# linnanwang/FastGen

Measured on AMD Instinct MI355X. Metric: images/sec at 4-step distilled (DMD2) sampling, higher is better.
Workload: dtype fp32 (tensors, accumulate) with split-bf16 x3 MFMA conv products; 1 GPU; EDM CIFAR-10 32x32 SongUNet (55.7M params) DMD2 4-step 'sde' sampling, batch=512 per GPU; global_batch=512, sample_steps=4, parallelism=replicas x1 (no data-path collective), graph=True

## Files before the change

### fastgen_amd/csrc/conv.h

```cpp
#pragma once
#include <hip/hip_runtime.h>

struct ConvArgs {
    const void* src1;
    const void* src2;
    int C1, C2;
    int Hs, Ws;
    int H, W;
    int B;
    const float2* ab;
    const void* wpack;
    const void* wpack_ws;
    const float* bias;
    const float* temb;
    int temb_stride;
    const void* resid;
    float scale;
    void* out;
    int Cout;
    float2* stats;
    int dbg;
    void* q_out;
    void* k_out;
    void* vt_out;
    const float* gate = nullptr;
    int gate_stride = 0;
    int act = 0;
    int heads = 0, head_dim = 0;
    size_t heads_lo_off = 0;
};

enum { PRO_NONE = 0, PRO_GN = 1, PRO_GN_SILU = 2 };
enum { RES_NONE = 0, RES_DOWN = 1, RES_UP = 2 };
enum { OUT_NHWC = 0, OUT_QKV = 1, OUT_TOK = 2, OUT_HEADS = 3 };

int launch_conv_fused(int dtype, int ks, int pro, int res, int outmode, const ConvArgs& a, hipStream_t stream);
int conv_stat_slots(int W);
bool conv_ws_supported(int dtype, int ks, int pro, int res, int outmode, const ConvArgs& a);
bool conv_ws_enabled();
int launch_conv_ws(int res, const ConvArgs& a, hipStream_t stream, bool prepare_only, int pro = PRO_GN_SILU);
bool conv_ws_shape_ok(int dtype, int cout, int cin, int res);
int launch_pack_conv_weights_ws(const float* w_oihw, void* wpack_ws, int cout, int cin, hipStream_t stream);
bool conv_x3ws_supported(int ks, int pro, int res, int outmode, const ConvArgs& a);
bool conv_x3ws_shape_ok(int cout, int cin, int res);
int conv_x3ws_stat_slots(int W);
int launch_conv_x3ws(int res, const ConvArgs& a, hipStream_t stream, bool prepare_only, int pro = PRO_GN_SILU);
int launch_pack_conv_weights_x3ws(const float* w_oihw, void* wpack_ws, int cout, int cin, hipStream_t stream);
int conv_launch_stat_slots(int dtype, int ks, int pro, int res, int outmode, const ConvArgs& a);
int launch_conv_ws_debug(const ConvArgs& a, int abl, hipStream_t stream);
int launch_conv_debug(int dtype, const ConvArgs& a, hipStream_t stream);
int conv_prepare_all(int dtype);
size_t conv_pack_elems(int cout, int cin, int ks);
int launch_pack_conv_weights(int dtype, const float* w_oihw, void* wpack, int cout, int cin, int ks, int qkv_perm,
                             hipStream_t stream);
```

### fastgen_amd/csrc/conv_ws3.hip

```cpp
#include "common.h"
#include "conv.h"

namespace {

constexpr int X3_NTHR = 768;
constexpr int X3_KC = 32;
constexpr int X3_PA = 16;
constexpr int X3_PLANE = 3072;
constexpr int X3_ABUF = 8 * X3_PLANE;
constexpr int X3_RING = 4;
constexpr int X3_HOFF = 128 * 512;
constexpr int X3_LDS = X3_HOFF + X3_RING * X3_ABUF;
constexpr int X3_STEPB = 9 * 2048;

template <int LOGW>
struct X3Geom {
    static constexpr int W = 1 << LOGW;
    static constexpr int TW = 16, TH = 8;
    static constexpr int TCOLS = W / TW;
    static constexpr int TPI = (W / TH) * TCOLS;
    static constexpr int HW_ = TW + 2, HH_ = TH + 2;
    static constexpr int HALO_PIX = HW_ * HH_;
    static constexpr int RS = HW_ * X3_PA;
};

__device__ __forceinline__ void x3_barrier() {
    asm volatile("s_waitcnt lgkmcnt(0)\n\ts_barrier" ::: "memory");
}

struct X3Frag {
    bf16x8 hi, lo;
};

template <int RES, int LOGW, int PRO>
__global__ __launch_bounds__(X3_NTHR) void conv3_x3ws_kernel(const ConvArgs a, const int ntiles) {
    using G = X3Geom<LOGW>;
    extern __shared__ __attribute__((aligned(16))) char smem[];
    char* const hbuf = smem;
    char* const ring = smem + X3_HOFF;

    const int tid = threadIdx.x;
    const int lane = tid & 63;
    const int wave = __builtin_amdgcn_readfirstlane(tid >> 6);
    const int Cin = a.C1 + a.C2;
    const int nchunk = Cin / X3_KC;
    const int G8 = (int)gridDim.x >> 3;
    const int wg = ((gridDim.x & 7) == 0) ? ((int)blockIdx.x & 7) * G8 + ((int)blockIdx.x >> 3) : (int)blockIdx.x;
    const int gstride = (int)gridDim.x;
    const int my_tiles = (ntiles - wg + gstride - 1) / gstride;
    const int S = my_tiles * nchunk;
    const int NSTEP = S + 3;
    const int H = a.H;

    if (wave < 8) {
        const int grp = wave >> 2, wl = wave & 3;
        const int col = lane & 15, g4 = lane >> 4;
        const size_t wstride = (size_t)nchunk * 9 * 1024;
        const __amdgpu_buffer_rsrc_t wrs = __builtin_amdgcn_make_buffer_rsrc(
            const_cast<__bf16*>(reinterpret_cast<const __bf16*>(a.wpack_ws) + (size_t)(grp * 8 + wl * 2) * wstride), 0, 0x7fffffff,
            0x00020000);
        const int wvoff = lane * 16;
        const int wsb = (int)(wstride * 2);
        auto load_w = [&](int byte_off) -> X3Frag {
            X3Frag f;
            f.hi = __builtin_bit_cast(bf16x8, __builtin_amdgcn_raw_buffer_load_b128(wrs, wvoff, byte_off, 0));
            f.lo = __builtin_bit_cast(bf16x8, __builtin_amdgcn_raw_buffer_load_b128(wrs, wvoff, byte_off + 1024, 0));
            return f;
        };
        X3Frag wq[3][2];
#pragma unroll
        for (int j = 0; j < 3; ++j)
#pragma unroll
            for (int nt = 0; nt < 2; ++nt) wq[j][nt] = load_w(nt * wsb + j * 2048);

        f32x4 acc[8][2];
#pragma unroll
        for (int m = 0; m < 8; ++m)
#pragma unroll
            for (int nt = 0; nt < 2; ++nt) acc[m][nt] = f32x4{0.f, 0.f, 0.f, 0.f};

        const int lane_off = g4 * X3_PLANE + col * X3_PA;
        const int dl0 = col * 512 + ((8 * wl + ((g4) ^ (col & 7))) << 4);
        const int dl1 = col * 512 + ((8 * wl + ((4 + g4) ^ (col & 7))) << 4);

        x3_barrier();
        int c = 0;
        for (int s = 0; s < NSTEP; ++s) {
            const int ls = s - 2 * grp;
            if (ls >= 0 && ls < S) {
                const char* abase = ring + (ls & 3) * X3_ABUF + lane_off;
                const int cn = (c + 1 == nchunk) ? 0 : c + 1;
                const int wcur = c * X3_STEPB;
                const int wnxt = (ls + 1 < S) ? cn * X3_STEPB : wcur;
                auto read_x = [&](int q, X3Frag (&xf)[2]) {
                    const int tap = q >> 2, m0 = 2 * (q & 3);
                    const int off = (tap / 3 + m0) * G::RS + (tap % 3) * X3_PA;
#pragma unroll
                    for (int m = 0; m < 2; ++m) {
                        xf[m].hi = *reinterpret_cast<const bf16x8*>(abase + off + m * G::RS);
                        xf[m].lo = *reinterpret_cast<const bf16x8*>(abase + off + m * G::RS + 4 * X3_PLANE);
                    }
                };
                auto mma12 = [&](int q, const X3Frag (&xf)[2]) {
                    const int tap = q >> 2, m0 = 2 * (q & 3);
                    const X3Frag(&wf)[2] = wq[tap % 3];
#pragma unroll
                    for (int m = 0; m < 2; ++m)
#pragma unroll
                        for (int nt = 0; nt < 2; ++nt)
                            acc[m0 + m][nt] = __builtin_amdgcn_mfma_f32_16x16x32_bf16(wf[nt].hi, xf[m].lo, acc[m0 + m][nt], 0, 0, 0);
#pragma unroll
                    for (int m = 0; m < 2; ++m)
#pragma unroll
                        for (int nt = 0; nt < 2; ++nt)
                            acc[m0 + m][nt] = __builtin_amdgcn_mfma_f32_16x16x32_bf16(wf[nt].lo, xf[m].hi, acc[m0 + m][nt], 0, 0, 0);
#pragma unroll
                    for (int m = 0; m < 2; ++m)
#pragma unroll
                        for (int nt = 0; nt < 2; ++nt)
                            acc[m0 + m][nt] = __builtin_amdgcn_mfma_f32_16x16x32_bf16(wf[nt].hi, xf[m].hi, acc[m0 + m][nt], 0, 0, 0);
                    if ((q & 3) != 3) return;
                    const int pn = (tap + 3 < 9) ? wcur + (tap + 3) * 2048 : wnxt + (tap + 3 - 9) * 2048;
#pragma unroll
                    for (int nt = 0; nt < 2; ++nt) wq[tap % 3][nt] = load_w(pn + nt * wsb);
                };
                X3Frag x0[2], x1[2];
                read_x(0, x0);
#pragma unroll
                for (int q = 0; q < 36; q += 2) {
                    read_x(q + 1, x1);
                    __builtin_amdgcn_sched_barrier(0);
                    mma12(q, x0);
                    __builtin_amdgcn_sched_barrier(0);
                    if (q + 2 < 36) read_x(q + 2, x0);
                    __builtin_amdgcn_sched_barrier(0);
                    mma12(q + 1, x1);
                    __builtin_amdgcn_sched_barrier(0);
                }
                if (c + 1 == nchunk) {
#pragma unroll
                    for (int m = 0; m < 8; ++m) {
                        *reinterpret_cast<f32x4*>(hbuf + m * 8192 + dl0) = acc[m][0];
                        *reinterpret_cast<f32x4*>(hbuf + m * 8192 + dl1) = acc[m][1];
                        acc[m][0] = f32x4{0.f, 0.f, 0.f, 0.f};
                        acc[m][1] = f32x4{0.f, 0.f, 0.f, 0.f};
                    }
                }
                c = cn;
            }
            x3_barrier();
        }
        return;
    }

    const int ptid = tid - 512;
    const int pw = wave - 8;
    const int oct = ptid & 3;
    const float* src1 = reinterpret_cast<const float*>(a.src1);
    const float* src2 = reinterpret_cast<const float*>(a.src2);
    int hdy[3], hdx[3], hlds[3];
#pragma unroll
    for (int i = 0; i < 3; ++i) {
        const int hq = min((ptid >> 2) + 64 * i, G::HALO_PIX - 1);
        const int hy = hq / G::HW_, hx = hq - hy * G::HW_;
        hdy[i] = hy - 1;
        hdx[i] = hx - 1;
        hlds[i] = oct * X3_PLANE + hy * G::RS + hx * X3_PA;
    }
    const bool third = (ptid >> 2) + 128 < G::HALO_PIX;

    auto tile_coord = [&](int t, int& n, int& slot, int& row0, int& col0) {
        n = t / G::TPI;
        slot = t - n * G::TPI;
        row0 = (slot / G::TCOLS) * G::TH;
        col0 = (slot % G::TCOLS) * G::TW;
    };

    struct Staged {
        f32x4 raw[3][2];
        float2 ab[8];
    };
    unsigned off1[3], off2[3];
    bool valid[3];
    const float2* abn = a.ab;
    auto tile_setup = [&](int t) __attribute__((always_inline)) {
        int n, slot, row0, col0;
        tile_coord(t, n, slot, row0, col0);
#pragma unroll
        for (int i = 0; i < 3; ++i) {
            const int y = row0 + hdy[i], x = col0 + hdx[i];
            valid[i] = (y >= 0) && (y < H) && (x >= 0) && (x < G::W) && (i < 2 || third);
            const int yc = min(max(y, 0), H - 1), xc = min(max(x, 0), G::W - 1);
            const int sy = (RES == RES_UP) ? (yc >> 1) : yc, sx = (RES == RES_UP) ? (xc >> 1) : xc;
            const unsigned pix = (unsigned)((n * a.Hs + sy) * a.Ws + sx);
            off1[i] = (pix * (unsigned)a.C1 + oct * 8) * 4u;
            off2[i] = (pix * (unsigned)a.C2 + oct * 8) * 4u;
        }
        abn = a.ab + (size_t)n * Cin;
    };
    auto stage_load = [&](Staged& st, int t, int c32) __attribute__((always_inline)) {
        if (c32 == 0) tile_setup(t);
        const bool first = c32 * X3_KC < a.C1;
        const char* base = first ? reinterpret_cast<const char*>(src1) + c32 * (X3_KC * 4)
                                 : reinterpret_cast<const char*>(src2) + (c32 * X3_KC - a.C1) * 4;
#pragma unroll
        for (int i = 0; i < 3; ++i) {
            const char* p = base + (first ? off1[i] : off2[i]);
            st.raw[i][0] = *reinterpret_cast<const f32x4*>(p);
            st.raw[i][1] = *reinterpret_cast<const f32x4*>(p + 16);
        }
        if (PRO == PRO_NONE) return;
        const float2* p = abn + c32 * X3_KC + oct * 8;
#pragma unroll
        for (int j = 0; j < 8; j += 2) {
            const f32x4 q = *reinterpret_cast<const f32x4*>(p + j);
            st.ab[j] = make_float2(q[0], q[1]);
            st.ab[j + 1] = make_float2(q[2], q[3]);
        }
    };
    auto stage_store = [&](const Staged& st, char* abuf) __attribute__((always_inline)) {
#pragma unroll
        for (int i = 0; i < 3; ++i) {
            float v[8];
#pragma unroll
            for (int j = 0; j < 8; ++j) {
                v[j] = st.raw[i][j >> 2][j & 3];
                if (PRO != PRO_NONE) v[j] = silu_f<true>(fmaf(v[j], st.ab[j].x, st.ab[j].y));
            }
            bf16x8 hi, lo;
            split8(v, hi, lo);
            typedef __attribute__((ext_vector_type(4))) unsigned u32x4;
            u32x4 wh = __builtin_bit_cast(u32x4, hi), wl_ = __builtin_bit_cast(u32x4, lo);
#pragma unroll
            for (int j = 0; j < 4; ++j) {
                wh[j] = valid[i] ? wh[j] : 0u;
                wl_[j] = valid[i] ? wl_[j] : 0u;
            }
            if (i < 2 || third) {
                *reinterpret_cast<u32x4*>(abuf + hlds[i]) = wh;
                *reinterpret_cast<u32x4*>(abuf + hlds[i] + 4 * X3_PLANE) = wl_;
            }
        }
    };

    const int chq = lane & 31, psub = lane >> 5;
    float* const out = reinterpret_cast<float*>(a.out);
    const float* const resid = reinterpret_cast<const float*>(a.resid);
    const bool has_resid = __builtin_amdgcn_readfirstlane(resid != nullptr);
    auto retire_half = [&](int t, int half) __attribute__((always_inline)) {
        int n, slot, row0, col0;
        tile_coord(t, n, slot, row0, col0);
        const int co = half * 128 + chq * 4;
        f32x4 radd = {0.f, 0.f, 0.f, 0.f};
        if (a.bias) radd = *reinterpret_cast<const f32x4*>(a.bias + co);
        if (a.temb) radd += *reinterpret_cast<const f32x4*>(a.temb + (size_t)n * a.temb_stride + co);
        radd *= a.scale;
        const size_t tb = (((size_t)n * H + row0) * G::W + col0) * 256 + co;
        float ssum = 0.f, ssq = 0.f;
#pragma unroll 1
        for (int grp8 = 0; grp8 < 2; ++grp8) {
            f32x4 rr[8], dv[8];
            unsigned go[8];
#pragma unroll
            for (int j = 0; j < 8; ++j) {
                const int px = pw * 32 + 2 * (grp8 * 8 + j) + psub;
                go[j] = (unsigned)(((px >> 4) * G::W + (px & 15)) * 256);
                rr[j] = f32x4{0.f, 0.f, 0.f, 0.f};
                if (has_resid) rr[j] = *reinterpret_cast<const f32x4*>(resid + tb + go[j]);
                dv[j] = *reinterpret_cast<const f32x4*>(hbuf + px * 512 + ((chq ^ (px & 7)) << 4));
            }
#pragma unroll
            for (int j = 0; j < 8; ++j) {
                f32x4 v;
#pragma unroll
                for (int e = 0; e < 4; ++e) v[e] = fmaf(dv[j][e], a.scale, radd[e]);
                if (has_resid) {
#pragma unroll
                    for (int e = 0; e < 4; ++e) v[e] = fmaf(rr[j][e], a.scale, v[e]);
                }
                *reinterpret_cast<f32x4*>(out + tb + go[j]) = v;
                ssum += (v[0] + v[1]) + (v[2] + v[3]);
                ssq += (v[0] * v[0] + v[1] * v[1]) + (v[2] * v[2] + v[3] * v[3]);
            }
        }
        ssum += __shfl_xor(ssum, 32);
        ssq += __shfl_xor(ssq, 32);
        if (a.stats && psub == 0) a.stats[(((size_t)n * G::TPI + slot) * 4 + pw) * 64 + half * 32 + chq] = make_float2(ssum, ssq);
    };

    auto advance = [&](int& t, int& cc) {
        if (++cc == nchunk) {
            cc = 0;
            t += gstride;
        }
    };
    Staged st;
    int t1 = wg, c1 = 0;
    stage_load(st, t1, c1);
    stage_store(st, ring);
    advance(t1, c1);
    x3_barrier();
    int sa = 0;
    for (int s = 0; s < NSTEP; ++s) {
        const bool more = s + 1 < S;
        if (more) stage_load(st, t1, c1);
        if (sa == 0 && s >= nchunk && s <= S) retire_half(wg + (s / nchunk - 1) * gstride, 0);
        if (sa == 2 % nchunk && s - 2 >= nchunk && s - 2 <= S && (s - 2) % nchunk == 0) retire_half(wg + ((s - 2) / nchunk - 1) * gstride, 1);
        if (more) {
            stage_store(st, ring + ((s + 1) & 3) * X3_ABUF);
            advance(t1, c1);
        }
        if (++sa == nchunk) sa = 0;
        x3_barrier();
    }
}

__global__ void pack_conv_weights_x3ws_kernel(const float* __restrict__ w, __bf16* __restrict__ out, int cout, int cin) {
    const size_t total = (size_t)cout * cin * 9;
    const int nstep = cin / X3_KC;
    for (size_t idx = (size_t)blockIdx.x * blockDim.x + threadIdx.x; idx < total; idx += (size_t)gridDim.x * blockDim.x) {
        size_t t = idx;
        const int j = t % 8; t /= 8;
        const int lane = t % 64; t /= 64;
        const int tap = t % 9; t /= 9;
        const int step = t % nstep; t /= nstep;
        const int n16 = (int)t;
        const int co = n16 * 16 + (lane & 15);
        const int ci = step * X3_KC + 8 * (lane >> 4) + j;
        const float v = w[((size_t)co * cin + ci) * 9 + tap];
        const __bf16 hi = (__bf16)v;
        const size_t o = (idx / 512) * 1024 + (idx % 512);
        out[o] = hi;
        out[o + 512] = (__bf16)(v - (float)hi);
    }
}

int g_x3_cus[16] = {};

template <int RES, int LOGW, int PRO>
int launch_x3_one(const ConvArgs& a, hipStream_t stream, bool prepare_only) {
    using G = X3Geom<LOGW>;
    auto kern = conv3_x3ws_kernel<RES, LOGW, PRO>;
    int dev = 0;
    if (hipGetDevice(&dev) != hipSuccess || dev < 0 || dev >= 16) return (int)hipErrorInvalidDevice;
    static bool attr_done[16] = {};
    if (!attr_done[dev]) {
        hipError_t e = hipFuncSetAttribute(reinterpret_cast<const void*>(kern), hipFuncAttributeMaxDynamicSharedMemorySize, X3_LDS);
        if (e != hipSuccess) return (int)e;
        attr_done[dev] = true;
    }
    if (!g_x3_cus[dev]) {
        int n = 0;
        if (hipDeviceGetAttribute(&n, hipDeviceAttributeMultiprocessorCount, dev) != hipSuccess || n <= 0) return (int)hipErrorUnknown;
        g_x3_cus[dev] = n;
    }
    if (prepare_only) return 0;
    const int ntiles = a.B * G::TPI;
    const int grid = ntiles < g_x3_cus[dev] ? ntiles : g_x3_cus[dev];
    hipLaunchKernelGGL(kern, dim3(grid), dim3(X3_NTHR), X3_LDS, stream, a, ntiles);
    return (int)hipGetLastError();
}

}

int conv_x3ws_stat_slots(int W) { return (W == 32 ? X3Geom<5>::TPI : X3Geom<4>::TPI) * 4; }

bool conv_x3ws_shape_ok(int cout, int cin, int res) { return cout == 256 && (res == 32 || res == 16) && (cin % X3_KC) == 0 && cin / X3_KC >= 4; }

bool conv_x3ws_supported(int ks, int pro, int res, int outmode, const ConvArgs& a) {
    const int cin = a.C1 + a.C2;
    const size_t src_bytes = (size_t)a.B * a.Hs * a.Ws * (size_t)(a.C1 > a.C2 ? a.C1 : a.C2) * 4;
    if (src_bytes >= (1ull << 32)) return false;
    if (ks != 3 || outmode != OUT_NHWC || a.H != a.W || !conv_x3ws_shape_ok(a.Cout, cin, a.W) || (a.C1 % X3_KC) || !a.wpack_ws) return false;
    if (pro == PRO_NONE) return res == RES_NONE && a.Hs == a.H && a.Ws == a.W;
    return pro == PRO_GN_SILU && (res == RES_NONE || res == RES_UP) && a.ab != nullptr;
}

int launch_conv_x3ws(int res, const ConvArgs& a, hipStream_t stream, bool prepare_only, int pro) {
    if (pro == PRO_NONE) {
        if (res != RES_NONE) return (int)hipErrorInvalidValue;
        return a.W == 32 ? launch_x3_one<RES_NONE, 5, PRO_NONE>(a, stream, prepare_only) : launch_x3_one<RES_NONE, 4, PRO_NONE>(a, stream, prepare_only);
    }
    if (a.W == 32)
        return res == RES_UP ? launch_x3_one<RES_UP, 5, PRO_GN_SILU>(a, stream, prepare_only) : launch_x3_one<RES_NONE, 5, PRO_GN_SILU>(a, stream, prepare_only);
    return res == RES_UP ? launch_x3_one<RES_UP, 4, PRO_GN_SILU>(a, stream, prepare_only) : launch_x3_one<RES_NONE, 4, PRO_GN_SILU>(a, stream, prepare_only);
}

int launch_pack_conv_weights_x3ws(const float* w_oihw, void* wpack_ws, int cout, int cin, hipStream_t stream) {
    const size_t total = (size_t)cout * cin * 9;
    const int grid = (int)((total + 255) / 256 < 4096 ? (total + 255) / 256 : 4096);
    hipLaunchKernelGGL(pack_conv_weights_x3ws_kernel, dim3(grid), dim3(256), 0, stream, w_oihw, (__bf16*)wpack_ws, cout, cin);
    return (int)hipGetLastError();
}
```

### fastgen_amd/csrc/engine.hip

```cpp
#include <hip/hip_runtime.h>

#include <cmath>
#include <cstdarg>
#include <cstdio>
#include <cstdlib>
#include <cstring>
#include <string>
#include <map>
#include <vector>

#include "../../include/fastgen_amd.h"
#include "common.h"
#include "adm.h"
#include "edm2.h"
#include "conv.h"
#include "misc.h"

namespace {

thread_local std::string g_err;

int fail(int code, const char* fmt, ...) {
    char buf[512];
    va_list ap;
    va_start(ap, fmt);
    vsnprintf(buf, sizeof buf, fmt, ap);
    va_end(ap);
    g_err = buf;
    return code;
}

#define HIP_TRY(expr)                                                                                          \
    do {                                                                                                       \
        hipError_t e_ = (hipError_t)(expr);                                                                    \
        if (e_ != hipSuccess) return fail(FG_EHIP, "%s failed: %s (%s:%d)", #expr, hipGetErrorString(e_), __FILE__, __LINE__); \
    } while (0)

struct Param {
    std::string name;
    int ndim = 0;
    int64_t shape[4] = {1, 1, 1, 1};
    int64_t numel = 0;
    const float* ptr = nullptr;
    float* grad = nullptr;
};

enum Kind { K_STEM, K_BLOCK, K_AUX_NORM, K_AUX_CONV };

struct Block {
    std::string key;
    Kind kind = K_BLOCK;
    int cin = 0, cout = 0, res_in = 0, res_out = 0;
    bool up = false, down = false, attn = false, has_skip = false, is_dec = false;
    int skip_c = 0;
    int temb_off = 0;
    int norm0_w = -1, norm0_b = -1, conv0_w = -1, conv0_b = -1, aff_w = -1, aff_b = -1, norm1_w = -1, norm1_b = -1,
        conv1_w = -1, conv1_b = -1, skip_w = -1, skip_b = -1, norm2_w = -1, norm2_b = -1, qkv_w = -1, qkv_b = -1,
        proj_w = -1, proj_b = -1, w = -1, b = -1;
    void *p_conv0 = nullptr, *p_conv1 = nullptr, *p_skip = nullptr, *p_qkv = nullptr, *p_proj = nullptr;
    void *p_conv0_ws = nullptr, *p_conv1_ws = nullptr;
    int tap = -1;
    float* qkv_bias = nullptr;
    void* p_aux = nullptr;
    void* p_stem = nullptr;
};

struct Arena {
    char* base = nullptr;
    size_t off = 0, cap = 0;
    bool dry = false;
    void* take(size_t bytes) {
        off = (off + 255) & ~(size_t)255;
        void* p = dry ? nullptr : base + off;
        off += bytes;
        return p;
    }
    template <typename T>
    T* get(size_t n) {
        return reinterpret_cast<T*>(take(n * sizeof(T)));
    }
};

struct Act {
    void* p = nullptr;
    float2* st = nullptr;
    int slots = 0;
};

struct AdmWs {
    float *e2 = nullptr, *lab = nullptr;
    float2* part = nullptr;
    std::vector<float*> skip;
    float *xa = nullptr, *xb = nullptr, *h = nullptr, *s = nullptr, *t1 = nullptr, *qkv = nullptr, *a = nullptr;
};
struct AdmNet;

struct Workspace {
    AdmWs adm;
    float *coef, *emb0, *emb1, *emb, *temb;
    float2 *ab0, *ab1, *ab2;
    float2 *mr0 = nullptr, *mr1 = nullptr, *mr2 = nullptr;
    void* a1d = nullptr;
    DropArgs drop;
    std::vector<Act> skip;
    Act xa, xb, h, xattn;
    void *sbuf, *aout, *pool;
    void *cvt1, *cvt2;
    void *q, *k, *vt;
    float *x, *x_pred, *eps;
    double* tl;
    uint64_t* seed;
};

// ... 485 lines not shown
        if (hipEventCreate(&e0) != hipSuccess || hipEventCreate(&e1) != hipSuccess) return (int)hipErrorUnknown;
        (void)hipEventRecord(e0, s);
    }
    const int rc = launch_conv_fused(h->cmode, ks, pro, res, outmode, a, s);
    if (timed) {
        (void)hipEventRecord(e1, s);
        h->prof_ev.push_back(e0);
        h->prof_ev.push_back(e1);
        h->prof_flops += 2.0 * a.B * a.H * a.W * (double)a.Cout * 9.0 * (a.C1 + a.C2);
    }
    return rc;
}

const float kSkipScale = (float)std::sqrt(0.5);
const float kBlockEps = 1e-6f;

int norm_coeffs(int dtype, const Act& x1, int c1, const Act& x2, int c2, const float* gamma, const float* beta, float2* ab,
                int B, int hw, hipStream_t s, float2* mr = nullptr) {
    if (x1.st && (!c2 || x2.st))
        HIP_TRY(launch_gn_finalize(x1.st, c1, x1.slots, c2 ? x2.st : nullptr, c2, c2 ? x2.slots : 0, gamma, beta, kBlockEps, ab, B, hw, s, mr));
    else
        HIP_TRY(launch_gn_coeffs(dtype, x1.p, c1, c2 ? x2.p : nullptr, c2, gamma, beta, kBlockEps, ab, B, hw, s, mr));
    return FG_OK;
}

void use_stash(Workspace& w, const BlockStash& st) {
    w.h.p = st.h;
    w.ab0 = st.ab0, w.ab1 = st.ab1, w.mr0 = st.mr0, w.mr1 = st.mr1;
    w.a1d = st.a1d;
    w.drop.block = st.index;
    if (st.xattn) {
        w.xattn.p = st.xattn;
        w.ab2 = st.ab2, w.mr2 = st.mr2;
        w.q = st.q, w.k = st.k, w.vt = st.vt, w.aout = st.aout;
    }
}
int block_index(const fg_edm* h, const Block* b) {
    for (size_t i = 0; i < h->blocks.size(); ++i)
        if (h->blocks[i] == b) return (int)i;
    return -1;
}

int run_block(fg_edm* h, const Block& b, const Act& x1, int c1, const Act& x2, int c2, const float* temb, Act& out, int B,
              Workspace& w, hipStream_t s) {
    if (c1 + c2 != b.cin) return fail(FG_EINVAL, "%s: got %d+%d input channels, expected %d", b.key.c_str(), c1, c2, b.cin);
    const int hw_in = b.res_in * b.res_in, hw = b.res_out * b.res_out;
    const int res_mode = b.down ? RES_DOWN : (b.up ? RES_UP : RES_NONE);
    const int slots = conv_stat_slots(b.res_out);
    int rc;
    if ((rc = norm_coeffs(h->dtype, x1, c1, x2, c2, h->P(b.norm0_w), h->P(b.norm0_b), w.ab0, B, hw_in, s, w.mr0))) return rc;
    ConvArgs a{};
    a.src1 = x1.p; a.src2 = c2 ? x2.p : nullptr; a.C1 = c1; a.C2 = c2;
    a.Hs = a.Ws = b.res_in; a.H = a.W = b.res_out; a.B = B;
    a.ab = w.ab0; a.wpack = b.p_conv0; a.wpack_ws = b.p_conv0_ws; a.bias = h->P(b.conv0_b);
    a.temb = temb + b.temb_off; a.temb_stride = h->temb_total;
    a.resid = nullptr; a.scale = 1.0f; a.out = w.h.p; a.Cout = b.cout; a.stats = w.h.st;
    if (b.down && !c2) {
        HIP_TRY(launch_gn_silu_pool(h->dtype, x1.p, w.ab0, w.pool, B, b.res_out, b.res_out, c1, s));
        a.src1 = w.pool; a.Hs = a.Ws = b.res_out; a.ab = nullptr;
        w.h.slots = conv_launch_stat_slots(h->cmode, 3, PRO_NONE, RES_NONE, OUT_NHWC, a);
        HIP_TRY(conv_launch(h, 3, PRO_NONE, RES_NONE, OUT_NHWC, a, s));
    } else {
        w.h.slots = conv_launch_stat_slots(h->cmode, 3, PRO_GN_SILU, res_mode, OUT_NHWC, a);
        HIP_TRY(conv_launch(h, 3, PRO_GN_SILU, res_mode, OUT_NHWC, a, s));
    }
    const void* resid = x1.p;
    if (b.has_skip) {
        ConvArgs k{};
        k.src1 = x1.p; k.src2 = c2 ? x2.p : nullptr; k.C1 = c1; k.C2 = c2;
        k.Hs = k.Ws = b.res_in; k.H = k.W = b.res_out; k.B = B;
        k.wpack = b.p_skip; k.bias = h->P(b.skip_b); k.scale = 1.0f; k.out = w.sbuf; k.Cout = b.cout;
        HIP_TRY(conv_launch(h, 1, PRO_NONE, res_mode, OUT_NHWC, k, s));
        resid = w.sbuf;
    }
    HIP_TRY(launch_gn_finalize(w.h.st, b.cout, w.h.slots, nullptr, 0, 0, h->P(b.norm1_w), h->P(b.norm1_b), kBlockEps, w.ab1, B, hw, s, w.mr1));
    Act& x_mid = b.attn ? w.xattn : out;
    ConvArgs d{};
    d.src1 = w.h.p; d.C1 = b.cout; d.Hs = d.Ws = d.H = d.W = b.res_out; d.B = B;
    d.ab = w.ab1; d.wpack = b.p_conv1; d.wpack_ws = b.p_conv1_ws; d.bias = h->P(b.conv1_b);
    d.resid = resid; d.scale = kSkipScale; d.out = x_mid.p; d.Cout = b.cout; d.stats = x_mid.st;
    if (w.a1d) {
        HIP_TRY(launch_gn_act(h->dtype, 0, w.h.p, b.cout, nullptr, 0, w.ab1, w.a1d, B, b.res_out, 0, s, w.drop));
        d.src1 = w.a1d; d.ab = nullptr;
        x_mid.slots = conv_launch_stat_slots(h->cmode, 3, PRO_NONE, RES_NONE, OUT_NHWC, d);
        HIP_TRY(conv_launch(h, 3, PRO_NONE, RES_NONE, OUT_NHWC, d, s));
    } else {
        x_mid.slots = conv_launch_stat_slots(h->cmode, 3, PRO_GN_SILU, RES_NONE, OUT_NHWC, d);
        HIP_TRY(conv_launch(h, 3, PRO_GN_SILU, RES_NONE, OUT_NHWC, d, s));
    }
    if (b.attn) {
        HIP_TRY(launch_gn_finalize(x_mid.st, b.cout, x_mid.slots, nullptr, 0, 0, h->P(b.norm2_w), h->P(b.norm2_b), kBlockEps, w.ab2, B, hw, s, w.mr2));
        ConvArgs q{};
        q.src1 = x_mid.p; q.C1 = b.cout; q.Hs = q.Ws = q.H = q.W = b.res_out; q.B = B;
        q.ab = w.ab2; q.wpack = b.p_qkv; q.bias = b.qkv_bias; q.scale = 1.0f; q.Cout = 3 * b.cout;
        q.q_out = w.q; q.k_out = w.k; q.vt_out = w.vt;
        HIP_TRY(conv_launch(h, 1, PRO_GN, RES_NONE, OUT_QKV, q, s));
        HIP_TRY(launch_attention(h->cmode, w.q, w.k, w.vt, w.aout, B, hw, s));
        ConvArgs p{};
        p.src1 = w.aout; p.C1 = b.cout; p.Hs = p.Ws = p.H = p.W = b.res_out; p.B = B;
        p.wpack = b.p_proj; p.bias = h->P(b.proj_b); p.resid = x_mid.p; p.scale = kSkipScale; p.out = out.p; p.Cout = b.cout;
        p.stats = out.st;
        HIP_TRY(conv_launch(h, 1, PRO_NONE, RES_NONE, OUT_NHWC, p, s));
        out.slots = slots;
    }
    return FG_OK;
}

// ... 81 lines not shown
        if (eps) {
            *e = eps + (size_t)i * total;
        } else {
            HIP_TRY(launch_randn(w.eps, total, 0, (uint64_t)i, w.seed, s));
            *e = w.eps;
        }
        return FG_OK;
    };
    if (loop == FG_LOOP_MEANFLOW) {
        for (int i = 0; i < steps; ++i) {
            const double* r = (type == FG_SAMPLE_SDE) ? w.tl + steps : w.tl + i + 1;
            int rc = run_forward(h, w.x, w.tl + i, 0, r, 0, labels, w.x_pred, B, w, s);
            if (rc) return rc;
            const bool renoise = type == FG_SAMPLE_SDE && t_list[i + 1] > 0;
            float* dst = (i == steps - 1 && !renoise) ? out : w.x;
            HIP_TRY(launch_meanflow_update(w.x, w.x_pred, w.tl, i, type == FG_SAMPLE_SDE ? -1 : i + 1, dst, total, s));
            if (renoise) {
                const float* e = nullptr;
                if ((rc = sde_noise(i, &e))) return rc;
                HIP_TRY(launch_forward_process(w.x, e, 0.0, w.tl, i + 1, sched, w.x, total, s));
            }
        }
        return FG_OK;
    }
    for (int i = 0; i < steps; ++i) {
        float* pred = (i == steps - 1) ? out : w.x_pred;
        int rc = run_forward(h, w.x, w.tl + i, 0, w.tl + steps, 0, labels, pred, B, w, s);
        if (rc) return rc;
        if (t_list[i + 1] > 0) {
            const float* e = nullptr;
            if (type == FG_SAMPLE_SDE) {
                if ((rc = sde_noise(i, &e))) return rc;
            } else {
                HIP_TRY(launch_x0_to_eps(w.x, pred, 0.0, w.tl, i, sched, 1e-6, w.eps, total, s));
                e = w.eps;
            }
            HIP_TRY(launch_forward_process(pred, e, 0.0, w.tl, i + 1, sched, w.x, total, s));
        }
    }
    return FG_OK;
}

int ensure_device_state(fg_edm* h) {
    if (h->device_ready) return FG_OK;
    int rc;
    const size_t tsz = h->dtype ? 2 : 4;
    for (Block* b : h->blocks) {
        if ((rc = h->alloc(&b->p_conv0, conv_pack_elems(b->cout, b->cin, 3) * tsz))) return rc;
        if ((rc = h->alloc(&b->p_conv1, conv_pack_elems(b->cout, b->cout, 3) * tsz))) return rc;
        const bool x3 = h->cmode == FG_DTYPE_BF16X3;
        if ((x3 ? conv_x3ws_shape_ok(b->cout, b->cin, b->res_out) : conv_ws_shape_ok(h->cmode, b->cout, b->cin, b->res_out)) && !b->down &&
            (rc = h->alloc(&b->p_conv0_ws, conv_pack_elems(b->cout, b->cin, 3) * tsz)))
            return rc;
        if ((x3 ? conv_x3ws_shape_ok(b->cout, b->cout, b->res_out) : conv_ws_shape_ok(h->cmode, b->cout, b->cout, b->res_out)) &&
            (rc = h->alloc(&b->p_conv1_ws, conv_pack_elems(b->cout, b->cout, 3) * tsz)))
            return rc;
        if (b->has_skip && (rc = h->alloc(&b->p_skip, conv_pack_elems(b->cout, b->cin, 1) * tsz))) return rc;
        if (b->attn) {
            if ((rc = h->alloc(&b->p_qkv, conv_pack_elems(3 * b->cout, b->cout, 1) * tsz))) return rc;
            if ((rc = h->alloc(&b->p_proj, conv_pack_elems(b->cout, b->cout, 1) * tsz))) return rc;
            if ((rc = h->alloc((void**)&b->qkv_bias, sizeof(float) * 3 * b->cout))) return rc;
        }
    }
    for (Block& b : h->enc)
        if (b.kind == K_STEM && stem_supported(b.res_out, b.cin, b.cout))
            if ((rc = h->alloc(&b.p_stem, stem_pack_elems() * tsz))) return rc;
    for (Block& b : h->dec)
        if (b.kind == K_AUX_CONV && aux_head_supported(h->cmode, b.res_out, b.cin, b.cout))
            if ((rc = h->alloc(&b.p_aux, aux_pack_elems(b.cin) * tsz))) return rc;
    if ((rc = h->alloc((void**)&h->aff_w, sizeof(float) * (size_t)h->temb_total * h->emb_ch))) return rc;
    if ((rc = h->alloc((void**)&h->aff_b, sizeof(float) * (size_t)h->temb_total))) return rc;
    const int half = h->noise_ch / 2;
    std::vector<float> fr(half);
    for (int j = 0; j < half; ++j) fr[j] = powf(1.0f / 10000.0f, (float)j / (float)(half - 1));
    if ((rc = h->alloc((void**)&h->freqs, sizeof(float) * half))) return rc;
    HIP_TRY(hipMemcpy(h->freqs, fr.data(), sizeof(float) * half, hipMemcpyHostToDevice));
    if (conv_prepare_all(h->cmode) != 0) return fail(FG_EHIP, "hipFuncSetAttribute(dynamic LDS) failed");
    if (launch_attention(h->cmode, nullptr, nullptr, nullptr, nullptr, 1, 256, nullptr) != 0) return fail(FG_EHIP, "attention prepare failed");
    h->device_ready = true;
    return FG_OK;
}

#include "engine_adm.inc"

}

extern "C" {

const char* fg_last_error(void) { return g_err.c_str(); }
const char* fg_version(void) { return "fastgen_amd 0.1 gfx950"; }

int fg_edm_create(const fg_edm_config* cfg, fg_edm** out) {
    if (!cfg || !out) return fail(FG_EINVAL, "null argument");
    if (cfg->num_levels < 1 || cfg->num_levels > FG_MAX_LEVELS || cfg->num_attn_resolutions < 0 ||
        cfg->num_attn_resolutions > FG_MAX_LEVELS)
        return fail(FG_EINVAL, "bad num_levels / num_attn_resolutions");
    if (cfg->compute_dtype != FG_DTYPE_F32 && cfg->compute_dtype != FG_DTYPE_BF16 && cfg->compute_dtype != FG_DTYPE_BF16X3)
        return fail(FG_EINVAL, "bad compute_dtype");
    if ((cfg->drop_precond & ~3) || (cfg->schedule != FG_SCHEDULE_EDM && cfg->schedule != FG_SCHEDULE_RF) ||
        (cfg->r_timestep & ~1))
        return fail(FG_EINVAL, "bad r_timestep / drop_precond / schedule");
    if (cfg->model_channels <= 0 || cfg->model_channels % 16 || cfg->channel_mult_noise < 1 || cfg->channel_mult_emb < 1)
        return fail(FG_EINVAL, "bad channel configuration");
    if (cfg->model_type != FG_MODEL_SONGUNET && cfg->model_type != FG_MODEL_DHARIWAL) return fail(FG_EINVAL, "bad model_type");
    fg_edm* h = new fg_edm();
    h->cfg = *cfg;
// ... 18 lines not shown
    h->noise_ch = cfg->model_channels * cfg->channel_mult_noise;
    h->cond_ch = h->noise_ch * (cfg->r_timestep ? 2 : 1);
    build_layout(h);
    rc = check_supported(h);
    if (rc) {
        delete h;
        return rc;
    }
    *out = h;
    return FG_OK;
}

void fg_edm_destroy(fg_edm* h) {
    if (!h) return;
    h->sampler.release();
    for (hipEvent_t e : h->prof_ev) (void)hipEventDestroy(e);
    delete h->adm;
    delete h;
}

int fg_edm_num_params(const fg_edm* h) { return h ? (int)h->params.size() : 0; }

int fg_edm_param_info(const fg_edm* h, int index, const char** name, int* ndim, int64_t shape[4]) {
    return param_info(h, index, name, ndim, shape);
}

int fg_edm_bind_param(fg_edm* h, const char* name, const float* device_ptr, int64_t numel) {
    return bind_param(h, name, device_ptr, numel);
}

int fg_edm_pack_weights(fg_edm* h, void* stream) {
    if (!h) return fail(FG_EINVAL, "null handle");
    hipStream_t s = (hipStream_t)stream;
    auto unused = [&](int i) {
        const std::string& n = h->params[i].name;
        return (n == "model.map_augment.weight" && (h->adm || !h->augment)) || n.rfind("model.logvar_linear", 0) == 0;
    };
    int rc;
    if (h->adm) {
        if ((rc = h->check_bound(unused))) return rc;
        ++h->pack_epoch;
        if ((rc = adm_pack_weights(h, s))) return rc;
        h->sampler.graph.drop();
        h->packed = true;
        return FG_OK;
    }
    if ((rc = ensure_device_state(h)) || (rc = h->check_bound(unused))) return rc;
    ++h->pack_epoch;
    for (Block* b : h->blocks) {
        HIP_TRY(launch_pack_conv_weights(h->cmode, h->P(b->conv0_w), b->p_conv0, b->cout, b->cin, 3, 0, s));
        HIP_TRY(launch_pack_conv_weights(h->cmode, h->P(b->conv1_w), b->p_conv1, b->cout, b->cout, 3, 0, s));
        if (h->cmode == FG_DTYPE_BF16X3) {
            if (b->p_conv0_ws) HIP_TRY(launch_pack_conv_weights_x3ws(h->P(b->conv0_w), b->p_conv0_ws, b->cout, b->cin, s));
            if (b->p_conv1_ws) HIP_TRY(launch_pack_conv_weights_x3ws(h->P(b->conv1_w), b->p_conv1_ws, b->cout, b->cout, s));
        } else {
            if (b->p_conv0_ws) HIP_TRY(launch_pack_conv_weights_ws(h->P(b->conv0_w), b->p_conv0_ws, b->cout, b->cin, s));
            if (b->p_conv1_ws) HIP_TRY(launch_pack_conv_weights_ws(h->P(b->conv1_w), b->p_conv1_ws, b->cout, b->cout, s));
        }
        if (b->has_skip) HIP_TRY(launch_pack_conv_weights(h->cmode, h->P(b->skip_w), b->p_skip, b->cout, b->cin, 1, 0, s));
        if (b->attn) {
            HIP_TRY(launch_pack_conv_weights(h->cmode, h->P(b->qkv_w), b->p_qkv, 3 * b->cout, b->cout, 1, 1, s));
            HIP_TRY(launch_pack_conv_weights(h->cmode, h->P(b->proj_w), b->p_proj, b->cout, b->cout, 1, 0, s));
            for (int plane = 0; plane < 3; ++plane)
                HIP_TRY(hipMemcpy2DAsync(b->qkv_bias + plane * b->cout, sizeof(float), h->P(b->qkv_b) + plane,
                                         3 * sizeof(float), sizeof(float), b->cout, hipMemcpyDeviceToDevice, s));
        }
        HIP_TRY(hipMemcpyAsync(h->aff_w + (size_t)b->temb_off * h->emb_ch, h->P(b->aff_w),
                               sizeof(float) * (size_t)b->cout * h->emb_ch, hipMemcpyDeviceToDevice, s));
        HIP_TRY(hipMemcpyAsync(h->aff_b + b->temb_off, h->P(b->aff_b), sizeof(float) * b->cout, hipMemcpyDeviceToDevice, s));
    }
    for (Block& b : h->enc)
        if (b.kind == K_STEM && b.p_stem) HIP_TRY(launch_pack_stem_weights(h->dtype, h->P(b.w), b.p_stem, b.cin, s));
    for (Block& b : h->dec)
        if (b.kind == K_AUX_CONV && b.p_aux) HIP_TRY(launch_pack_aux_weights(h->cmode, h->P(b.w), b.p_aux, b.cin, b.cout, s));
    h->sampler.graph.drop();
    h->packed = true;
    return FG_OK;
}

size_t fg_edm_workspace_bytes(const fg_edm* h, int batch) {
    if (!h || batch <= 0) return 0;
    Arena A;
    A.dry = true;
    Workspace w;
    return plan_workspace(h, batch, A, w);
}

int fg_edm_forward(fg_edm* h, const float* x_t, const double* t, const double* r, const float* class_labels, float* out,
                   float* emb_out, int batch, void* workspace, size_t workspace_bytes, void* stream) {
    if (!h || !x_t || !t || !out) return fail(FG_EINVAL, "null argument");
    if (r && !h->cfg.r_timestep) return fail(FG_EINVAL, "r_noise_labels provided, but r_timestep is not set");
    if (!r && h->cfg.r_timestep) return fail(FG_EINVAL, "this network was built with r_timestep: r is required");
    if (!h->packed) return fail(FG_ENOTREADY, "weights are not packed (call fg_edm_pack_weights)");
    if (out == x_t) return fail(FG_EINVAL, "out must not alias x_t");
    Workspace w;
    int rc = setup_ws(plan_workspace, h, batch, workspace, workspace_bytes, w);
    if (rc) return rc;
    hipStream_t s = (hipStream_t)stream;
    rc = run_forward(h, x_t, t, 1, r, 1, class_labels, out, batch, w, s);
    if (rc) return rc;
    if (emb_out) HIP_TRY(hipMemcpyAsync(emb_out, w.emb, sizeof(float) * (size_t)batch * h->emb_ch, hipMemcpyDeviceToDevice, s));
    return FG_OK;
}

int fg_edm_num_feature_taps(const fg_edm* h) { return h ? h->num_taps : 0; }

// ... 475 lines not shown
```

Measured before the change: 2716 img/s.

## Use sub-pixel 2x2 decomposition for upsample+3x3 conv at 32x32

For the nearest-upsample followed by 3x3 conv at 32x32 outputs, precomputes four phase-specific 2x2 kernels by summing the 3x3 taps that fall on the same low-res source pixel. The kernel then convolves the 16x16 source directly with 4 taps instead of 9, cutting MFMA work and weight traffic for that layer by more than half. Each tile covers one output phase, and writes are strided by 2 in the output. This adds a separate weight pack buffer and a new template path. Folding taps before the bf16 hi/lo split changes rounding slightly.

New measurement: 2749 img/s (median of 6 runs). +1.2%, better.

```diff
diff --git a/fastgen_amd/csrc/conv.h b/fastgen_amd/csrc/conv.h
--- a/fastgen_amd/csrc/conv.h
+++ b/fastgen_amd/csrc/conv.h
@@ -28,6 +28,7 @@
     int act = 0;
     int heads = 0, head_dim = 0;
     size_t heads_lo_off = 0;
+    const void* wpack_sp = nullptr;
 };
 
 enum { PRO_NONE = 0, PRO_GN = 1, PRO_GN_SILU = 2 };
@@ -46,6 +47,8 @@
 int conv_x3ws_stat_slots(int W);
 int launch_conv_x3ws(int res, const ConvArgs& a, hipStream_t stream, bool prepare_only, int pro = PRO_GN_SILU);
 int launch_pack_conv_weights_x3ws(const float* w_oihw, void* wpack_ws, int cout, int cin, hipStream_t stream);
+size_t conv_x3sp_pack_elems(int cout, int cin);
+int launch_pack_conv_weights_x3sp(const float* w_oihw, void* wpack_sp, int cout, int cin, hipStream_t stream);
 int conv_launch_stat_slots(int dtype, int ks, int pro, int res, int outmode, const ConvArgs& a);
 int launch_conv_ws_debug(const ConvArgs& a, int abl, hipStream_t stream);
 int launch_conv_debug(int dtype, const ConvArgs& a, hipStream_t stream);
diff --git a/fastgen_amd/csrc/conv_ws3.hip b/fastgen_amd/csrc/conv_ws3.hip
--- a/fastgen_amd/csrc/conv_ws3.hip
+++ b/fastgen_amd/csrc/conv_ws3.hip
@@ -11,7 +11,8 @@
 constexpr int X3_RING = 4;
 constexpr int X3_HOFF = 128 * 512;
 constexpr int X3_LDS = X3_HOFF + X3_RING * X3_ABUF;
-constexpr int X3_STEPB = 9 * 2048;
+
+constexpr int X3_SUB = 3;
 
 template <int LOGW>
 struct X3Geom {
@@ -35,6 +36,12 @@
 template <int RES, int LOGW, int PRO>
 __global__ __launch_bounds__(X3_NTHR) void conv3_x3ws_kernel(const ConvArgs a, const int ntiles) {
     using G = X3Geom<LOGW>;
+    constexpr bool SUB = RES == X3_SUB;
+    constexpr int NTAP = SUB ? 4 : 9;
+    constexpr int NR = SUB ? 2 : 3;
+    constexpr int SB = (SUB ? 16 : 9) * 2048;
+    constexpr int LW = G::W / 2, LTCOLS = LW / G::TW;
+    static_assert(!SUB || LOGW == 5, "the sub-pixel form is built for 32x32 outputs only");
     extern __shared__ __attribute__((aligned(16))) char smem[];
     char* const hbuf = smem;
     char* const ring = smem + X3_HOFF;
@@ -55,7 +62,7 @@
     if (wave < 8) {
         const int grp = wave >> 2, wl = wave & 3;
         const int col = lane & 15, g4 = lane >> 4;
-        const size_t wstride = (size_t)nchunk * 9 * 1024;
+        const size_t wstride = (size_t)nchunk * (SB / 2);
         const __amdgpu_buffer_rsrc_t wrs = __builtin_amdgcn_make_buffer_rsrc(
             const_cast<__bf16*>(reinterpret_cast<const __bf16*>(a.wpack_ws) + (size_t)(grp * 8 + wl * 2) * wstride), 0, 0x7fffffff,
             0x00020000);
@@ -67,11 +74,13 @@
             f.lo = __builtin_bit_cast(bf16x8, __builtin_amdgcn_raw_buffer_load_b128(wrs, wvoff, byte_off + 1024, 0));
             return f;
         };
-        X3Frag wq[3][2];
-#pragma unroll
-        for (int j = 0; j < 3; ++j)
-#pragma unroll
-            for (int nt = 0; nt < 2; ++nt) wq[j][nt] = load_w(nt * wsb + j * 2048);
+        auto phase_of = [&](int t) { return SUB ? (t % G::TPI) & 3 : 0; };
+        int tk = wg;
+        X3Frag wq[NR][2];
+#pragma unroll
+        for (int j = 0; j < NR; ++j)
+#pragma unroll
+            for (int nt = 0; nt < 2; ++nt) wq[j][nt] = load_w(nt * wsb + phase_of(tk) * (4 * 2048) + j * 2048);
 
         f32x4 acc[8][2];
 #pragma unroll
@@ -88,13 +97,16 @@
         for (int s = 0; s < NSTEP; ++s) {
             const int ls = s - 2 * grp;
             if (ls >= 0 && ls < S) {
-                const char* abase = ring + (ls & 3) * X3_ABUF + lane_off;
+                const int ph = phase_of(tk);
+                const char* abase = ring + (ls & 3) * X3_ABUF + lane_off + (SUB ? (ph >> 1) * G::RS + (ph & 1) * X3_PA : 0);
                 const int cn = (c + 1 == nchunk) ? 0 : c + 1;
-                const int wcur = c * X3_STEPB;
-                const int wnxt = (ls + 1 < S) ? cn * X3_STEPB : wcur;
+                const int wcur = c * SB + ph * (4 * 2048);
+                const int wnxt = (ls + 1 < S) ? cn * SB + phase_of(cn ? tk : tk + gstride) * (4 * 2048)
+                                              : wcur;
                 auto read_x = [&](int q, X3Frag (&xf)[2]) {
                     const int tap = q >> 2, m0 = 2 * (q & 3);
-                    const int off = (tap / 3 + m0) * G::RS + (tap % 3) * X3_PA;
+                    const int ty = SUB ? tap >> 1 : tap / 3, tx = SUB ? tap & 1 : tap % 3;
+                    const int off = (ty + m0) * G::RS + tx * X3_PA;
 #pragma unroll
                     for (int m = 0; m < 2; ++m) {
                         xf[m].hi = *reinterpret_cast<const bf16x8*>(abase + off + m * G::RS);
@@ -103,7 +115,7 @@
                 };
                 auto mma12 = [&](int q, const X3Frag (&xf)[2]) {
                     const int tap = q >> 2, m0 = 2 * (q & 3);
-                    const X3Frag(&wf)[2] = wq[tap % 3];
+                    const X3Frag(&wf)[2] = wq[tap % NR];
 #pragma unroll
                     for (int m = 0; m < 2; ++m)
 #pragma unroll
@@ -120,19 +132,19 @@
                         for (int nt = 0; nt < 2; ++nt)
                             acc[m0 + m][nt] = __builtin_amdgcn_mfma_f32_16x16x32_bf16(wf[nt].hi, xf[m].hi, acc[m0 + m][nt], 0, 0, 0);
                     if ((q & 3) != 3) return;
-                    const int pn = (tap + 3 < 9) ? wcur + (tap + 3) * 2048 : wnxt + (tap + 3 - 9) * 2048;
-#pragma unroll
-                    for (int nt = 0; nt < 2; ++nt) wq[tap % 3][nt] = load_w(pn + nt * wsb);
+                    const int pn = (tap + NR < NTAP) ? wcur + (tap + NR) * 2048 : wnxt + (tap + NR - NTAP) * 2048;
+#pragma unroll
+                    for (int nt = 0; nt < 2; ++nt) wq[tap % NR][nt] = load_w(pn + nt * wsb);
                 };
                 X3Frag x0[2], x1[2];
                 read_x(0, x0);
 #pragma unroll
-                for (int q = 0; q < 36; q += 2) {
+                for (int q = 0; q < 4 * NTAP; q += 2) {
                     read_x(q + 1, x1);
                     __builtin_amdgcn_sched_barrier(0);
                     mma12(q, x0);
                     __builtin_amdgcn_sched_barrier(0);
-                    if (q + 2 < 36) read_x(q + 2, x0);
+                    if (q + 2 < 4 * NTAP) read_x(q + 2, x0);
                     __builtin_amdgcn_sched_barrier(0);
                     mma12(q + 1, x1);
                     __builtin_amdgcn_sched_barrier(0);
@@ -146,6 +158,7 @@
                         acc[m][1] = f32x4{0.f, 0.f, 0.f, 0.f};
                     }
                 }
+                if (cn == 0) tk += gstride;
                 c = cn;
             }
             x3_barrier();
@@ -172,8 +185,9 @@
     auto tile_coord = [&](int t, int& n, int& slot, int& row0, int& col0) {
         n = t / G::TPI;
         slot = t - n * G::TPI;
-        row0 = (slot / G::TCOLS) * G::TH;
-        col0 = (slot % G::TCOLS) * G::TW;
+        const int ts = SUB ? slot >> 2 : slot;
+        row0 = (ts / (SUB ? LTCOLS : G::TCOLS)) * G::TH;
+        col0 = (ts % (SUB ? LTCOLS : G::TCOLS)) * G::TW;
     };
 
     struct Staged {
@@ -186,11 +200,13 @@
     auto tile_setup = [&](int t) __attribute__((always_inline)) {
         int n, slot, row0, col0;
         tile_coord(t, n, slot, row0, col0);
+        constexpr int SW = SUB ? LW : G::W;
+        const int SH = SUB ? a.Hs : H;
 #pragma unroll
         for (int i = 0; i < 3; ++i) {
             const int y = row0 + hdy[i], x = col0 + hdx[i];
-            valid[i] = (y >= 0) && (y < H) && (x >= 0) && (x < G::W) && (i < 2 || third);
-            const int yc = min(max(y, 0), H - 1), xc = min(max(x, 0), G::W - 1);
+            valid[i] = (y >= 0) && (y < SH) && (x >= 0) && (x < SW) && (i < 2 || third);
+            const int yc = min(max(y, 0), SH - 1), xc = min(max(x, 0), SW - 1);
             const int sy = (RES == RES_UP) ? (yc >> 1) : yc, sx = (RES == RES_UP) ? (xc >> 1) : xc;
             const unsigned pix = (unsigned)((n * a.Hs + sy) * a.Ws + sx);
             off1[i] = (pix * (unsigned)a.C1 + oct * 8) * 4u;
@@ -255,7 +271,8 @@
         if (a.bias) radd = *reinterpret_cast<const f32x4*>(a.bias + co);
         if (a.temb) radd += *reinterpret_cast<const f32x4*>(a.temb + (size_t)n * a.temb_stride + co);
         radd *= a.scale;
-        const size_t tb = (((size_t)n * H + row0) * G::W + col0) * 256 + co;
+        const int ph = SUB ? slot & 3 : 0, ps = SUB ? 2 : 1;
+        const size_t tb = (((size_t)n * H + ps * row0 + (ph >> 1)) * G::W + ps * col0 + (ph & 1)) * 256 + co;
         float ssum = 0.f, ssq = 0.f;
 #pragma unroll 1
         for (int grp8 = 0; grp8 < 2; ++grp8) {
@@ -264,7 +281,7 @@
 #pragma unroll
             for (int j = 0; j < 8; ++j) {
                 const int px = pw * 32 + 2 * (grp8 * 8 + j) + psub;
-                go[j] = (unsigned)(((px >> 4) * G::W + (px & 15)) * 256);
+                go[j] = (unsigned)((ps * (px >> 4) * G::W + ps * (px & 15)) * 256);
                 rr[j] = f32x4{0.f, 0.f, 0.f, 0.f};
                 if (has_resid) rr[j] = *reinterpret_cast<const f32x4*>(resid + tb + go[j]);
                 dv[j] = *reinterpret_cast<const f32x4*>(hbuf + px * 512 + ((chq ^ (px & 7)) << 4));
@@ -335,6 +352,33 @@
     }
 }
 
+__global__ void pack_conv_weights_x3sp_kernel(const float* __restrict__ w, __bf16* __restrict__ out, int cout, int cin) {
+    const size_t total = (size_t)cout * cin * 16;
+    const int nstep = cin / X3_KC;
+    for (size_t idx = (size_t)blockIdx.x * blockDim.x + threadIdx.x; idx < total; idx += (size_t)gridDim.x * blockDim.x) {
+        size_t t = idx;
+        const int j = t % 8; t /= 8;
+        const int lane = t % 64; t /= 64;
+        const int tap = t % 4; t /= 4;
+        const int ph = t % 4; t /= 4;
+        const int step = t % nstep; t /= nstep;
+        const int n16 = (int)t;
+        const int co = n16 * 16 + (lane & 15);
+        const int ci = step * X3_KC + 8 * (lane >> 4) + j;
+        const int py = ph >> 1, px = ph & 1, ty = tap >> 1, tx = tap & 1;
+        const int ky0 = ty ? 1 + py : 0, ky1 = ty ? 2 : py, kx0 = tx ? 1 + px : 0, kx1 = tx ? 2 : px;
+        const float* wp = w + ((size_t)co * cin + ci) * 9;
+        double acc = 0.0;
+        for (int ky = ky0; ky <= ky1; ++ky)
+            for (int kx = kx0; kx <= kx1; ++kx) acc += (double)wp[ky * 3 + kx];
+        const float v = (float)acc;
+        const __bf16 hi = (__bf16)v;
+        const size_t o = (idx / 512) * 1024 + (idx % 512);
+        out[o] = hi;
+        out[o + 512] = (__bf16)(v - (float)hi);
+    }
+}
+
 int g_x3_cus[16] = {};
 
 template <int RES, int LOGW, int PRO>
@@ -381,8 +425,20 @@
         if (res != RES_NONE) return (int)hipErrorInvalidValue;
         return a.W == 32 ? launch_x3_one<RES_NONE, 5, PRO_NONE>(a, stream, prepare_only) : launch_x3_one<RES_NONE, 4, PRO_NONE>(a, stream, prepare_only);
     }
-    if (a.W == 32)
-        return res == RES_UP ? launch_x3_one<RES_UP, 5, PRO_GN_SILU>(a, stream, prepare_only) : launch_x3_one<RES_NONE, 5, PRO_GN_SILU>(a, stream, prepare_only);
+    if (a.W == 32 && res == RES_UP) {
+        if (prepare_only) {
+            const int rc = launch_x3_one<X3_SUB, 5, PRO_GN_SILU>(a, stream, true);
+            return rc ? rc : launch_x3_one<RES_UP, 5, PRO_GN_SILU>(a, stream, true);
+        }
+        if (a.wpack_sp) {
+            if (a.Hs * 2 != a.H || a.Ws * 2 != a.W) return (int)hipErrorInvalidValue;
+            ConvArgs s = a;
+            s.wpack_ws = a.wpack_sp;
+            return launch_x3_one<X3_SUB, 5, PRO_GN_SILU>(s, stream, false);
+        }
+        return launch_x3_one<RES_UP, 5, PRO_GN_SILU>(a, stream, false);
+    }
+    if (a.W == 32) return launch_x3_one<RES_NONE, 5, PRO_GN_SILU>(a, stream, prepare_only);
     return res == RES_UP ? launch_x3_one<RES_UP, 4, PRO_GN_SILU>(a, stream, prepare_only) : launch_x3_one<RES_NONE, 4, PRO_GN_SILU>(a, stream, prepare_only);
 }
 
@@ -392,3 +448,13 @@
     hipLaunchKernelGGL(pack_conv_weights_x3ws_kernel, dim3(grid), dim3(256), 0, stream, w_oihw, (__bf16*)wpack_ws, cout, cin);
     return (int)hipGetLastError();
 }
+
+size_t conv_x3sp_pack_elems(int cout, int cin) { return (size_t)cout * cin * 16 * 2; }
+
+int launch_pack_conv_weights_x3sp(const float* w_oihw, void* wpack_sp, int cout, int cin, hipStream_t stream) {
+    if (cout % 16 || cin % X3_KC) return (int)hipErrorInvalidValue;
+    const size_t total = (size_t)cout * cin * 16;
+    const int grid = (int)((total + 255) / 256 < 4096 ? (total + 255) / 256 : 4096);
+    hipLaunchKernelGGL(pack_conv_weights_x3sp_kernel, dim3(grid), dim3(256), 0, stream, w_oihw, (__bf16*)wpack_sp, cout, cin);
+    return (int)hipGetLastError();
+}
diff --git a/fastgen_amd/csrc/engine.hip b/fastgen_amd/csrc/engine.hip
--- a/fastgen_amd/csrc/engine.hip
+++ b/fastgen_amd/csrc/engine.hip
@@ -59,6 +59,7 @@
         proj_w = -1, proj_b = -1, w = -1, b = -1;
     void *p_conv0 = nullptr, *p_conv1 = nullptr, *p_skip = nullptr, *p_qkv = nullptr, *p_proj = nullptr;
     void *p_conv0_ws = nullptr, *p_conv1_ws = nullptr;
+    void* p_conv0_sp = nullptr;
     int tap = -1;
     float* qkv_bias = nullptr;
     void* p_aux = nullptr;
@@ -650,7 +651,7 @@
     ConvArgs a{};
     a.src1 = x1.p; a.src2 = c2 ? x2.p : nullptr; a.C1 = c1; a.C2 = c2;
     a.Hs = a.Ws = b.res_in; a.H = a.W = b.res_out; a.B = B;
-    a.ab = w.ab0; a.wpack = b.p_conv0; a.wpack_ws = b.p_conv0_ws; a.bias = h->P(b.conv0_b);
+    a.ab = w.ab0; a.wpack = b.p_conv0; a.wpack_ws = b.p_conv0_ws; a.wpack_sp = b.p_conv0_sp; a.bias = h->P(b.conv0_b);
     a.temb = temb + b.temb_off; a.temb_stride = h->temb_total;
     a.resid = nullptr; a.scale = 1.0f; a.out = w.h.p; a.Cout = b.cout; a.stats = w.h.st;
     if (b.down && !c2) {
@@ -838,6 +839,9 @@
         if ((x3 ? conv_x3ws_shape_ok(b->cout, b->cin, b->res_out) : conv_ws_shape_ok(h->cmode, b->cout, b->cin, b->res_out)) && !b->down &&
             (rc = h->alloc(&b->p_conv0_ws, conv_pack_elems(b->cout, b->cin, 3) * tsz)))
             return rc;
+        if (x3 && b->up && b->res_out == 32 && conv_x3ws_shape_ok(b->cout, b->cin, b->res_out) &&
+            (rc = h->alloc(&b->p_conv0_sp, conv_x3sp_pack_elems(b->cout, b->cin) * 2)))
+            return rc;
         if ((x3 ? conv_x3ws_shape_ok(b->cout, b->cout, b->res_out) : conv_ws_shape_ok(h->cmode, b->cout, b->cout, b->res_out)) &&
             (rc = h->alloc(&b->p_conv1_ws, conv_pack_elems(b->cout, b->cout, 3) * tsz)))
             return rc;
@@ -962,6 +966,7 @@
         HIP_TRY(launch_pack_conv_weights(h->cmode, h->P(b->conv1_w), b->p_conv1, b->cout, b->cout, 3, 0, s));
         if (h->cmode == FG_DTYPE_BF16X3) {
             if (b->p_conv0_ws) HIP_TRY(launch_pack_conv_weights_x3ws(h->P(b->conv0_w), b->p_conv0_ws, b->cout, b->cin, s));
+            if (b->p_conv0_sp) HIP_TRY(launch_pack_conv_weights_x3sp(h->P(b->conv0_w), b->p_conv0_sp, b->cout, b->cin, s));
             if (b->p_conv1_ws) HIP_TRY(launch_pack_conv_weights_x3ws(h->P(b->conv1_w), b->p_conv1_ws, b->cout, b->cout, s));
         } else {
             if (b->p_conv0_ws) HIP_TRY(launch_pack_conv_weights_ws(h->P(b->conv0_w), b->p_conv0_ws, b->cout, b->cin, s));
```
